# dy-tea/zpaq-v

Hardware: AMD Instinct MI355X
Metric: MB/s (comp+decomp) on level-2 64KiB blocks (higher is better)
Workload: dtype int32; 1 GPU; level 2 (ICM16+ISSE16+ISSE16), 8192 x 65536 B blocks per GPU (C5's per-GPU share of 65536 blocks over 8 GPUs), one segment per block, classes b mod 4 = zeros/uniform/markov-text/periodic (SURVEY 8(d) generator, block b of the global batch on rank b mod N); blocks_per_gpu=8192, block_bytes=65536, level=2, parallelism=block b -> gpu b mod 1, no collective

## Files before the change

### include/zpaq_hip.h

```cpp
#ifndef ZPAQ_HIP_H
#define ZPAQ_HIP_H

#include <stddef.h>
#include <stdint.h>

#ifdef __cplusplus
extern "C" {
#endif

#define ZPQ_OK 0
#define ZPQ_E_NODEVICE (-1)
#define ZPQ_E_ARG (-2)
#define ZPQ_E_HEADER (-3)
#define ZPQ_E_TOOBIG (-4)
#define ZPQ_E_MIX_M0 (-5)
#define ZPQ_E_NOMEM (-6)
#define ZPQ_E_OVERFLOW (-7)
#define ZPQ_E_VMSTEPS (-8)
#define ZPQ_E_INTERNAL (-9)
#define ZPQ_E_CLOSED (-10)

#define ZPQ_VM_STEP_CAP (1u << 20)

#define ZPQ_FLAG_PP 1u
// ... 12 lines not shown
int zpq_model_ncomp(const zpq_model *);
uint64_t zpq_model_state_bytes(const zpq_model *);
int zpq_model_has_fast_path(const zpq_model *);

typedef struct zpq_ctx zpq_ctx;
int zpq_ctx_create(int device, zpq_ctx **out);
void zpq_ctx_destroy(zpq_ctx *);
int zpq_ctx_sync(zpq_ctx *);
void *zpq_ctx_stream(zpq_ctx *);
int zpq_ctx_device(const zpq_ctx *);
int zpq_ctx_set_state_budget(zpq_ctx *, uint64_t bytes);
int zpq_ctx_set_max_block_bytes(zpq_ctx *, uint64_t bytes);
int zpq_ctx_last_slots(const zpq_ctx *);
unsigned zpq_ctx_last_host_transfer(const zpq_ctx *);
unsigned zpq_ctx_last_line_store(const zpq_ctx *);
int zpq_ctx_resident_capacity(zpq_ctx *, const zpq_model *, uint32_t flags);
float zpq_ctx_last_kernel_ms(const zpq_ctx *);
const char *zpq_ctx_last_kernel_name(const zpq_ctx *);

int zpq_encode_blocks(zpq_ctx *, const zpq_model *, int nblocks, const uint8_t *in,
                      const uint64_t *in_off, uint32_t flags, uint8_t *out,
                      const uint64_t *out_off, uint32_t *out_len, int32_t *status);
int zpq_decode_blocks(zpq_ctx *, const zpq_model *, int nblocks, const uint8_t *in,
                      const uint64_t *in_off, uint32_t flags, uint8_t *out,
                      const uint64_t *out_off, uint32_t *out_len, uint32_t *consumed,
                      uint32_t *final_code, uint32_t *first_byte, int32_t *status);

void *zpq_host_alloc(size_t bytes);
void zpq_host_free(void *);

// ... 76 lines not shown
```

### zpaq-v_amd/binding.py

```python
import atexit
import ctypes as C
import os
import weakref

import numpy as np

HERE = os.path.dirname(os.path.abspath(__file__))
FLAG_PP = 1
FLAG_GENERIC = 2
FLAG_LANES = 8
FLAG_VMPIPE = 16
SET_LANES = 1
SET_PIPE = 4
SET_WAVES = 16
SET_VMWAVES = 64
_LIB = None
_LIVE_CTX = weakref.WeakSet()
_LIVE_PINNED = weakref.WeakSet()
_FINALIZING = False


def _shutdown():
    global _FINALIZING
    for ctx in list(_LIVE_CTX):
# ... 42 lines not shown
    L.zpq_model_state_bytes.restype = u64
    L.zpq_model_has_fast_path.argtypes = [vp]
    L.zpq_ctx_create.argtypes = [i32, vp]
    L.zpq_ctx_destroy.argtypes = [vp]
    L.zpq_ctx_sync.argtypes = [vp]
    L.zpq_ctx_stream.argtypes = [vp]
    L.zpq_ctx_stream.restype = vp
    L.zpq_ctx_set_state_budget.argtypes = [vp, u64]
    L.zpq_ctx_set_max_block_bytes.argtypes = [vp, u64]
    L.zpq_ctx_last_slots.argtypes = [vp]
    L.zpq_ctx_last_host_transfer.argtypes = [vp]
    L.zpq_ctx_last_host_transfer.restype = C.c_uint
    L.zpq_ctx_last_line_store.argtypes = [vp]
    L.zpq_ctx_last_line_store.restype = C.c_uint
    L.zpq_ctx_resident_capacity.argtypes = [vp, vp, u32]
    L.zpq_ctx_last_kernel_ms.argtypes = [vp]
    L.zpq_ctx_last_kernel_ms.restype = C.c_float
    L.zpq_ctx_last_kernel_name.argtypes = [vp]
    L.zpq_ctx_last_kernel_name.restype = C.c_char_p
    enc = [vp, vp, i32, vp, vp, u32, vp, vp, vp, vp]
    dec = [vp, vp, i32, vp, vp, u32, vp, vp, vp, vp, vp, vp, vp]
    L.zpq_encode_blocks.argtypes = enc
    L.zpq_encode_blocks_dev.argtypes = enc
    L.zpq_decode_blocks.argtypes = dec
    L.zpq_decode_blocks_dev.argtypes = dec
    L.zpq_host_alloc.argtypes = [C.c_size_t]
    L.zpq_host_alloc.restype = vp
    L.zpq_host_free.argtypes = [vp]
    L.zpq_encode_blocks_multi.argtypes = [vp, i32, vp, i32, vp, vp, u32, vp, vp, vp, vp]
    L.zpq_decode_blocks_multi.argtypes = [vp, i32, vp, i32, vp, vp, u32, vp, vp, vp, vp, vp, vp, vp]
# ... 198 lines not shown
    def last_kernel_name(self):
        return lib().zpq_ctx_last_kernel_name(self.h).decode()

    @property
    def last_slots(self):
        return lib().zpq_ctx_last_slots(self.h)

    @property
    def last_host_transfer(self):
        return lib().zpq_ctx_last_host_transfer(self.h)

    @property
    def last_line_store(self):
        return lib().zpq_ctx_last_line_store(self.h)

    def resident_capacity(self, model, flags=FLAG_PP):
        n = lib().zpq_ctx_resident_capacity(self.h, model.h, flags)
        if n < 0:
            raise ZpqError(n, "zpq_ctx_resident_capacity")
        return n

    def blockset_capacity(self, model, max_member_bytes=0, lanes=False, pipe=False, waves=False, vmwaves=False):
        n = lib().zpq_blockset_capacity_ex(self.h, model.h, max_member_bytes, _set_flags(lanes, pipe, waves, vmwaves))
        if n < 0:
            raise ZpqError(n, "zpq_blockset_capacity")
        return n

    def encode_blocks(self, model, blocks, flags=FLAG_PP, cap=None):
        nb = len(blocks)
        in_off = _offsets([len(b) for b in blocks])
# ... 291 lines not shown
```

### zpaq-v_amd/csrc/zpq_api.hip

```cpp
#include <hip/hip_runtime.h>
#include <stdio.h>
#include <stdlib.h>
#include <string.h>
#include <time.h>

#include <algorithm>
#include <exception>
#include <map>
#include <mutex>
#include <thread>
#include <unordered_set>
#include <vector>

#include "../../include/zpaq_hip.h"
#include "zpq_common.h"
#include "zpq_host.h"

#define ZPQ_SET_ALL (ZPQ_SET_LANES | ZPQ_SET_PIPE | ZPQ_SET_WAVES | ZPQ_SET_VMWAVES)

#define HIPCK(x)                                                              \
    do {                                                                      \
        hipError_t e_ = (x);                                                  \
        if (e_ != hipSuccess) {                                               \
            fprintf(stderr, "[zpaq_hip] %s failed: %s (%s:%d)\n", #x, hipGetErrorString(e_), __FILE__, __LINE__); \
// ... 18 lines not shown
            (void)hipGetLastError();
            q = nullptr;
            if (p) { (void)hipFree(p); p = nullptr; cap = 0; }
            if (hipMalloc(&q, want) != hipSuccess) {
                (void)hipGetLastError();
                want = n + 4096;
                if (hipMalloc(&q, want) != hipSuccess) { (void)hipGetLastError(); return ZPQ_E_NOMEM; }
            }
        }
        if (p) (void)hipFree(p);
        p = q;
        cap = want;
        return ZPQ_OK;
    }
    void release() { if (p) (void)hipFree(p); p = nullptr; cap = 0; }
    DevBuf() = default;
    DevBuf(const DevBuf &) = delete;
    DevBuf &operator=(const DevBuf &) = delete;
    ~DevBuf() { release(); }
};

struct BlockArrays {
    int n = 0;
    const uint8_t *in = nullptr; const uint64_t *in_off = nullptr;
    uint32_t flags = 0;
    uint8_t *out = nullptr; const uint64_t *out_off = nullptr;
    uint32_t *out_len = nullptr, *consumed = nullptr, *final_code = nullptr, *first_byte = nullptr;
    int32_t *status = nullptr;
    BlockArrays window(int b0, int b1) const
    {
// ... 78 lines not shown
};

struct zpq_ctx {
    int device = 0;
    int cus = 256;
    hipStream_t stream = nullptr;
    hipEvent_t ev0 = nullptr, ev1 = nullptr;
    bool ev_valid = false;
    int16_t *d_squash = nullptr, *d_stretch = nullptr, *d_dt2k = nullptr;
    uint32_t *d_dt = nullptr, *d_stretch_c = nullptr;
    uint8_t *d_ns = nullptr;
    std::map<uint64_t, DevModel> models;
    uint32_t sparse_cap = 0;
    uint32_t sparse_pct = 112;
    DevBuf slots;
    uint64_t budget = 0;
    int last_slots = 0;
    unsigned last_host = 0;
    uint32_t last_sp = 0;
    const char *last_name = "";
    StageSet one, pipe[2];
    hipStream_t s_h2d = nullptr, s_d2h = nullptr;
    uint32_t *h_gate = nullptr;
    std::mutex mu;
    std::vector<zpq_block *> children;
    std::vector<zpq_blockset *> sets;
    uint64_t set_bytes = 0;
    uint64_t pool_budget() const { return budget > set_bytes ? budget - set_bytes : 0; }
};

// ... 35 lines not shown
    const zpq_model *model = nullptr;
    int nmembers = 0;
    bool chain = false;
    uint32_t flags = 0;
    uint32_t sp = 0;
    DModel layout;
    uint8_t *slots = nullptr;
    uint64_t bytes = 0;
    std::vector<int32_t> failed;
    std::vector<uint8_t> fresh;
    std::vector<uint8_t> open;
};

static int ctx_init(zpq_ctx *c, const zpq::Tables &T);
static int set_max_block_bytes(zpq_ctx *c, uint64_t bytes);
extern "C" int zpq_ctx_create(int device, zpq_ctx **out) try
{
    if (!out) return ZPQ_E_ARG;
    *out = nullptr;
    int ndev = 0;
    if (hipGetDeviceCount(&ndev) != hipSuccess || ndev <= 0) return ZPQ_E_NODEVICE;
    if (device < 0 || device >= ndev) return ZPQ_E_ARG;
    int tst = ZPQ_OK;
    const zpq::Tables &T = zpq::tables(&tst);
    if (tst != ZPQ_OK) return tst;
    HIPCK(hipSetDevice(device));
    zpq_ctx *c = new (std::nothrow) zpq_ctx();
    if (!c) return ZPQ_E_NOMEM;
    c->device = device;
    const int rc = ctx_init(c, T);
// ... 1 lines not shown
    if (rc != ZPQ_OK) { zpq_ctx_destroy(c); return rc; }
    *out = c;
    return ZPQ_OK;
} ZPQ_CATCH(return ZPQ_E_INTERNAL)

static int ctx_init(zpq_ctx *c, const zpq::Tables &T)
{
    const int device = c->device;
    hipDeviceProp_t prop;
    if (hipGetDeviceProperties(&prop, device) == hipSuccess) c->cus = prop.multiProcessorCount;
    HIPCK(hipStreamCreateWithFlags(&c->stream, hipStreamNonBlocking));
    HIPCK(hipEventCreate(&c->ev0));
    HIPCK(hipEventCreate(&c->ev1));
    HIPCK(hipStreamCreateWithFlags(&c->s_h2d, hipStreamNonBlocking));
    HIPCK(hipStreamCreateWithFlags(&c->s_d2h, hipStreamNonBlocking));
    HIPCK(hipHostMalloc((void **)&c->h_gate, 64, hipHostMallocPortable | hipHostMallocMapped));
    *c->h_gate = 1;
    for (auto &ps : c->pipe) if (int rc = ps.create_events()) return rc;
    std::vector<int16_t> sq(4096), st(32768), d2(256);
    for (int i = 0; i < 4096; i++) sq[i] = (int16_t)T.squash[i];
    for (int i = 0; i < 32768; i++) st[i] = (int16_t)T.stretch[i];
    for (int i = 0; i < 256; i++) d2[i] = (int16_t)T.dt2k[i];
    HIPCK(hipMalloc((void **)&c->d_squash, 4096 * 2));
    HIPCK(hipMalloc((void **)&c->d_stretch, 32768 * 2));
    HIPCK(hipMalloc((void **)&c->d_dt2k, 256 * 2));
    HIPCK(hipMalloc((void **)&c->d_dt, 1024 * 4));
    HIPCK(hipMalloc((void **)&c->d_ns, 1024));
    HIPCK(hipMalloc((void **)&c->d_stretch_c, sizeof T.stretch_c));
    HIPCK(hipMemcpy(c->d_squash, sq.data(), 4096 * 2, hipMemcpyHostToDevice));
    HIPCK(hipMemcpy(c->d_stretch, st.data(), 32768 * 2, hipMemcpyHostToDevice));
// ... 9 lines not shown
        const int pct = ev ? atoi(ev) : 0;
        if (pct >= 101 && pct <= 400) c->sparse_pct = (uint32_t)pct;
    }
    set_max_block_bytes(c, 65536);
    return ZPQ_OK;
}

extern "C" void zpq_ctx_destroy(zpq_ctx *c) try
{
    {
        std::lock_guard<std::mutex> lk(g_reg_mu);
        if (!c || !live_set().erase(c)) return;
    }
    (void)hipSetDevice(c->device);
    if (c->stream) (void)hipStreamSynchronize(c->stream);
    {
        std::lock_guard<std::mutex> lk(g_reg_mu);
        for (zpq_block *b : c->children) {
            if (b->slot) (void)hipFree(b->slot);
            b->slot = nullptr;
            b->ctx = nullptr;
        }
        c->children.clear();
        for (zpq_blockset *bs : c->sets) {
            if (bs->slots) (void)hipFree(bs->slots);
            bs->slots = nullptr;
            bs->ctx = nullptr;
        }
        c->sets.clear();
        c->set_bytes = 0;
    }
    for (auto &kv : c->models) { (void)hipFree(kv.second.d_model); (void)hipFree(kv.second.d_img); }
    if (c->h_gate) (void)hipHostFree(c->h_gate);
    if (c->s_h2d) { (void)hipStreamSynchronize(c->s_h2d); (void)hipStreamDestroy(c->s_h2d); }
    if (c->s_d2h) { (void)hipStreamSynchronize(c->s_d2h); (void)hipStreamDestroy(c->s_d2h); }
    (void)hipFree(c->d_squash); (void)hipFree(c->d_stretch); (void)hipFree(c->d_dt2k);
    (void)hipFree(c->d_dt); (void)hipFree(c->d_ns); (void)hipFree(c->d_stretch_c);
    if (c->ev0) (void)hipEventDestroy(c->ev0);
    if (c->ev1) (void)hipEventDestroy(c->ev1);
    if (c->stream) (void)hipStreamDestroy(c->stream);
    delete c;
} ZPQ_CATCH(return)

extern "C" int zpq_ctx_sync(zpq_ctx *c) try
{
    if (!ctx_live(c)) return ZPQ_E_ARG;
    HIPCK(hipStreamSynchronize(c->stream));
    return ZPQ_OK;
} ZPQ_CATCH(return ZPQ_E_INTERNAL)
extern "C" int zpq_ctx_device(const zpq_ctx *c) { return ctx_live(c) ? c->device : -1; }
extern "C" void *zpq_ctx_stream(zpq_ctx *c) { return ctx_live(c) ? (void *)c->stream : nullptr; }
extern "C" int zpq_ctx_set_state_budget(zpq_ctx *c, uint64_t bytes) try
{
    if (!ctx_live(c)) return ZPQ_E_ARG;
    c->budget = bytes;
    return ZPQ_OK;
} ZPQ_CATCH(return ZPQ_E_INTERNAL)
extern "C" int zpq_ctx_set_max_block_bytes(zpq_ctx *c, uint64_t bytes) try
{
    if (!ctx_live(c)) return ZPQ_E_ARG;
    return set_max_block_bytes(c, bytes);
} ZPQ_CATCH(return ZPQ_E_INTERNAL)
static uint32_t line_store_cap(const zpq_ctx *c, uint64_t bytes)
{
    const uint64_t probes = 2 * (bytes + 2);
    uint64_t cap = (probes * c->sparse_pct + 99) / 100 + 16;
    cap = (cap + 3) & ~3ull;
    if (cap > (1ull << 25)) cap = 1ull << 25;
    return (uint32_t)cap;
}
static int set_max_block_bytes(zpq_ctx *c, uint64_t bytes)
{
    c->sparse_cap = line_store_cap(c, bytes);
    return ZPQ_OK;
}
// ... 20 lines not shown
    HIPCK(hipMalloc((void **)&dm.d_img, m->img.size() * 4 + 4));
    HIPCK(hipMemcpy(dm.d_model, &layout, sizeof(DModel), hipMemcpyHostToDevice));
    HIPCK(hipMemcpy(dm.d_img, m->img.data(), m->img.size() * 4, hipMemcpyHostToDevice));
    c->models[key] = dm;
    *out = dm;
    return ZPQ_OK;
}

struct BatchArgs {
    BlockArrays io;
    BatchExtras x;
    const uint32_t *gate_flag = nullptr;
    uint32_t gate_pos = 0;
    uint32_t *prog_counter = nullptr;
    uint32_t prog_pos = 0;
};

static bool request(const char *var, uint32_t flags, uint32_t bit)
{
    const char *ev = getenv(var);
    const bool env = ev && (ev[0] == '0' || ev[0] == '1');
    return env ? ev[0] == '1' : (flags & bit) != 0;
}
struct SparseKnobs {
    uint32_t forced_cap = 0;
    bool never = false, always = false;
};
static SparseKnobs sparse_knobs()
{
    SparseKnobs k;
// ... 147 lines not shown
    if (rc != ZPQ_OK) return rc;
    c->last_name = name;
    HIPCK(hipGetLastError());
    HIPCK(hipEventRecord(c->ev1, s));
    c->ev_valid = true;
    return ZPQ_OK;
}
static int launch_family(zpq_ctx *c, const DBatch &B, const Plan &P, int decode, hipStream_t s)
{
    return timed_launch(c, s, [&](const char **name) {
        *name = FAMILY[P.fam].name[decode];
        return FAMILY[P.fam].launch(&B, P, decode, s, name);
    });
}

static int run_batch(zpq_ctx *c, const zpq_model *m, int decode, const BatchArgs &a)
{
    const BlockArrays &io = a.io;
    if (!ctx_live(c)) return c ? ZPQ_E_CLOSED : ZPQ_E_ARG;
    if (!m) return ZPQ_E_ARG;
    if (io.n < 0) return ZPQ_E_ARG;
    if (io.n == 0) return ZPQ_OK;
    if (!io.in_off || !io.out_off || !io.out_len || !io.status) return ZPQ_E_ARG;
    if (a.x.own_slot && io.n != 1) return ZPQ_E_ARG;
    HIPCK(hipSetDevice(c->device));
    Plan P;
    int rc = plan_batch(c, m, io.flags, io.n, a.x.trace != nullptr, a.x.own_slot != nullptr, &P, decode);
    if (rc != ZPQ_OK) return rc;
    DevModel dm;
    rc = get_dev_model(c, m, P.M, P.sp, &dm);
    if (rc != ZPQ_OK) return rc;

    DBatch B = batch_base(c, dm, io);
    B.trace = a.x.trace; B.ntrace = a.x.ntrace; B.ctx_out = a.x.ctx_out;
    B.gate_flag = (P.fam == F_CHAIN && !decode) ? a.gate_flag : nullptr;
    B.gate_pos = a.gate_pos;
    if (a.gate_flag && !B.gate_flag) return ZPQ_E_INTERNAL;
    B.prog_counter = (P.fam == F_CHAIN && decode) ? a.prog_counter : nullptr;
    B.prog_pos = a.prog_pos;

    if (a.x.own_slot) {
        B.slots = a.x.own_slot;
    } else {
        rc = c->slots.ensure((size_t)P.nslots * P.M.slot_bytes + 256);
        if (rc != ZPQ_OK) return rc;
        B.slots = (uint8_t *)c->slots.p;
    }
    B.nslots = P.nslots;
    c->last_slots = P.nslots;
    c->last_sp = P.sp;
    c->last_host = 0;
    return launch_family(c, B, P, decode, c->stream);
}

extern "C" int zpq_encode_blocks_dev(zpq_ctx *c, const zpq_model *m, int nblocks, const uint8_t *in,
                                     const uint64_t *in_off, uint32_t flags, uint8_t *out,
                                     const uint64_t *out_off, uint32_t *out_len, int32_t *status) try
{
    BatchArgs a;
    a.io = block_arrays(nblocks, in, in_off, flags & 0xffu, out, out_off, out_len, status);
    return run_batch(c, m, 0, a);
} ZPQ_CATCH(return ZPQ_E_INTERNAL)

extern "C" int zpq_decode_blocks_dev(zpq_ctx *c, const zpq_model *m, int nblocks, const uint8_t *in,
                                     const uint64_t *in_off, uint32_t flags, uint8_t *out,
                                     const uint64_t *out_off, uint32_t *out_len, uint32_t *consumed,
                                     uint32_t *final_code, uint32_t *first_byte, int32_t *status) try
{
    BatchArgs a;
    a.io = block_arrays(nblocks, in, in_off, flags & 0xffu, out, out_off, out_len, status, consumed, final_code, first_byte);
    return run_batch(c, m, 1, a);
} ZPQ_CATCH(return ZPQ_E_INTERNAL)

static int stage_room(StageSet &S, int nb, size_t in_bytes, size_t out_bytes, size_t misc_bytes)
{
    int rc;
    const size_t offb = (size_t)(nb + 1) * 8, u32b = (size_t)nb * 4;
    if ((rc = S.in.ensure(in_bytes + 16)) || (rc = S.out.ensure(out_bytes + 16)) || (rc = S.inoff.ensure(offb)) ||
        (rc = S.outoff.ensure(offb)) || (rc = S.dstoff.ensure(offb)) || (rc = S.meta.ensure(u32b * 4)) || (rc = S.status.ensure(u32b)) ||
        (rc = S.misc.ensure(misc_bytes)) || (rc = S.ensure_host((size_t)nb)))
        return rc;
    return ZPQ_OK;
}
static void stage_offsets(StageSet &S, const BlockArrays &h)
{
// ... 570 lines not shown
    if (!ctx_live(c)) return c ? ZPQ_E_CLOSED : ZPQ_E_ARG;
    if (!m || nmembers < 1) return ZPQ_E_ARG;
    HIPCK(hipSetDevice(c->device));
    std::lock_guard<std::mutex> lk(c->mu);
    zpq_blockset *s = new (std::nothrow) zpq_blockset();
    if (!s) return ZPQ_E_NOMEM;
    s->chain = set_layout(c, m, max_member_bytes, &s->layout, &s->sp);
    s->flags = (uint32_t)zpq_blockset_resolve_flags(m, flags);
    const bool lanes = (s->flags & ZPQ_SET_LANES) != 0;
    s->nmembers = nmembers;
    s->bytes = (uint64_t)nmembers * s->layout.slot_bytes + 256;
    if (nmembers > set_capacity(c, s->layout, s->chain, lanes) || s->bytes > c->pool_budget()) { delete s; return ZPQ_E_NOMEM; }
    if (hipMalloc((void **)&s->slots, s->bytes) != hipSuccess) {
        (void)hipGetLastError();
        (void)hipStreamSynchronize(c->stream);
        c->slots.release();
        if (hipMalloc((void **)&s->slots, s->bytes) != hipSuccess) { (void)hipGetLastError(); delete s; return ZPQ_E_NOMEM; }
    }
    int rc = ZPQ_OK;
    if (s->chain || lanes) {
        DevModel dm;
        rc = get_dev_model(c, m, s->layout, s->sp, &dm);
        if (rc == ZPQ_OK) rc = zpq_launch_lanes_set_init(dm.d_model, dm.d_img, s->slots, nmembers, c->stream);
        if (rc == ZPQ_OK && (hipGetLastError() != hipSuccess || hipStreamSynchronize(c->stream) != hipSuccess)) rc = ZPQ_E_NODEVICE;
    }
    if (rc != ZPQ_OK) { (void)hipGetLastError(); (void)hipFree(s->slots); delete s; return rc; }
    s->failed.assign((size_t)nmembers, ZPQ_OK);
    s->fresh.assign((size_t)nmembers, 1);
    s->open.assign((size_t)nmembers, 0);
    s->ctx = c; s->model = m;
// ... 251 lines not shown
```

### zpaq-v_amd/csrc/zpq_chain.hip

```cpp
#include <hip/hip_runtime.h>
#include <stdlib.h>
#include <string.h>

#include <type_traits>
#include <vector>

#include "../../include/zpaq_hip.h"
#include "zpq_common.h"
#include "zpq_vm.h"
#include "zpq_host.h"
#include "zpq_chain_cfg.h"
#include "zpq_dev.h"

constexpr int CHAIN_G_DEFAULT = 8;
constexpr bool CHAIN_SPEC_ENC = true, CHAIN_SPEC_DEC = false;

namespace zpqc {

using namespace zpqdev;
__device__ __forceinline__ i32 mul24x(i32 a, i32 b) { return __mul24(a, b); }

__device__ __forceinline__ i32 row_shr1(i32 self)
{
    return __builtin_amdgcn_update_dpp(self, self, 0x111 , 0xf, 0xf, false);
// ... 136 lines not shown
                        const u32 cmi = cmk[i] & 0x7FFFFFu;
                        const i32 sti = stretch_of(cmi);
                        d32[i] = cmi | (((u32)sti & 0x1FFu) << 23);
                        d8[i] = (u8)(sti >> 9);
                    } else {
                        const u32 a0 = cmk[2 * i], a1 = cmk[2 * i + 1];
                        d32[i] = (a0 & 0xFFFFFu) | (a1 << 20);
                        d8[i] = (u8)((i32)a1 >> 12);
                    }
                }
            }
        } else {
            uint4 *z4 = reinterpret_cast<uint4 *>(slot);
            const u64 n16 = M.zero_bytes / 16;
            const uint4 zero = make_uint4(0, 0, 0, 0);
            for (u64 i = li; i < n16; i += G) z4[i] = zero;
            for (int c = 0; c < n; c++) {
                const DComp &cc = M.comp[c];
                u32 *d32 = reinterpret_cast<u32 *>(my + cfg.lds_off32[c]);
                if (cc.type == ZT_ICM) {
                    u8 *d8 = my + cfg.lds_off8[c];
                    for (int i = li; i < 256; i += G) {
                        const u32 cmi = B.img[i];
                        const i32 sti = stretch_of(cmi);
                        d32[i] = cmi | (((u32)sti & 0x1FFu) << 23);
                        d8[i] = (u8)(sti >> 9);
                    }
                }
                else if (cc.type == ZT_ISSE) {
                    u8 *d8 = my + cfg.lds_off8[c];
                    for (int i = li; i < 256; i += G) {
// ... 1230 lines not shown
```

### zpaq-v_amd/csrc/zpq_common.h

```cpp
#pragma once
#include <stdint.h>

#define ZPQ_MAX_HDR 4096
#define ZPQ_MAX_COMP 255

enum { ZT_NONE = 0, ZT_CONST = 1, ZT_CM = 2, ZT_ICM = 3, ZT_MATCH = 4, ZT_AVG = 5,
       ZT_MIX2 = 6, ZT_MIX = 7, ZT_ISSE = 8, ZT_SSE = 9 };

enum { ZF_ZERO = 0, ZF_CONST = 1, ZF_PATTERN = 2 };

struct DComp {
    int32_t type;
    int32_t a, b, c, limit;
    int32_t j, k, rate, mask;
    uint32_t cm_len, ht_len, a16_len;
    uint32_t cm_fill, cm_fill_val, cm_pat_len;
    uint32_t a16_fill;
    uint32_t sp_cap;
    uint64_t cm_off, ht_off, a16_off;
    uint64_t sp_tag_off, sp_line_off;
};

struct DCompScal {
    int32_t a, b, c, limit;
// ... 15 lines not shown
    uint64_t regs_off, r_off, scal_off, h_off, m_off;
    uint64_t zero_bytes;
    uint64_t slot_bytes;
    uint32_t img_words;
    uint32_t pad_;
    uint8_t header[ZPQ_MAX_HDR];
    DComp comp[ZPQ_MAX_COMP];
};

struct DBatch {
    const DModel *model;
    const uint32_t *img;
    uint8_t *slots;
    int32_t nslots, nblocks;
    uint32_t flags;
    uint32_t ntrace;
    const uint8_t *in;
    const uint64_t *in_off;
    uint8_t *out;
    const uint64_t *out_off;
    uint32_t *out_len;
    uint32_t *consumed;
    uint32_t *final_code;
    uint32_t *first_byte;
    int32_t *status;
    union {
        int32_t *trace;
        const int32_t *slot_map;
    };
    uint32_t *ctx_out;
    const int16_t *squash;
// ... 23 lines not shown
```

### zpaq-v_amd/csrc/zpq_host.h

```cpp
#pragma once
#include <hip/hip_runtime.h>
#include <stdint.h>

#include <atomic>
#include <vector>

#include "zpq_common.h"

namespace zpq {

struct Tables {
    int32_t squash[4096];
    int32_t stretch[32768];
    int32_t dt[1024];
    int32_t dt2k[256];
    uint8_t ns[1024];
    uint32_t stretch_c[2048 + 128];
};
const Tables &tables(int *status);
uint64_t tables_fnv(int which);

}

bool zpq_sparse_layout(const DModel &dense, uint32_t cap, DModel *out);
// ... 32 lines not shown
int zpq_gdec_shape_applies(const DModel *M);
int zpq_gpipe_applies(const DModel *M);
int zpq_gpipe_blocks_per_cu(const DModel *M);
int zpq_launch_gpipe(const DBatch *B, const DModel *hostM, int nslots, hipStream_t stream);
int zpq_gdec_applies(const DModel *M);
int zpq_gdec_blocks_per_cu(const DModel *M);
int zpq_launch_gdec(const DBatch *B, const DModel *hostM, int nslots, hipStream_t stream);
int zpq_vpipe_applies(const DModel *M);
int zpq_vpipe_blocks_per_cu(const DModel *M);
int zpq_launch_vpipe(const DBatch *B, const DModel *hostM, int nslots, hipStream_t stream);
int zpq_vdec_applies(const DModel *M);
int zpq_vdec_blocks_per_cu(const DModel *M);
int zpq_launch_vdec(const DBatch *B, const DModel *hostM, int nslots, hipStream_t stream);
int zpq_launch_wset(const DBatch *B, const DModel *hostM, int decode, hipStream_t stream, const char **name);
int zpq_launch_vset(const DBatch *B, const DModel *hostM, int decode, hipStream_t stream, const char **name);
int zpq_launch_sha1(const uint8_t *in, const uint64_t *beg, const uint64_t *end, int n, uint8_t *out20, hipStream_t stream);
}

void zpq_note_exception(const char *where) noexcept;
#define ZPQ_CATCH(on_error) catch (...) { zpq_note_exception(__func__); on_error; }

template <class R, class F> static inline R zpq_guard(R on_error, const char *where, F &&f) noexcept
{
    try { return f(); } catch (...) { zpq_note_exception(where); return on_error; }
}
template <class F> static inline void zpq_guard_v(const char *where, F &&f) noexcept
{
    try { f(); } catch (...) { zpq_note_exception(where); }
}
```

### zpaq-v_amd/csrc/zpq_pipe.hip

```cpp
#include <hip/hip_runtime.h>
#include <stdlib.h>
#include <string.h>

#include <type_traits>

#include "../../include/zpaq_hip.h"
#include "zpq_common.h"
#include "zpq_chain_cfg.h"
#include "zpq_dev.h"
#include "zpq_host.h"

namespace zpqp {

using namespace zpqc;
using namespace zpqdev;

__device__ __forceinline__ bool gate_wait(const uint32_t *flag)
{
    u32 tries = 0;
    while (__hip_atomic_load(flag, __ATOMIC_ACQUIRE, __HIP_MEMORY_SCOPE_SYSTEM) == 0u) {
        __builtin_amdgcn_s_sleep(64);
        if (++tries > (1u << 22)) return false;
    }
    return true;
// ... 867 lines not shown
                    reinterpret_cast<u32 *>(blk_lds + cfg.lds_off32[0])[i] = cmi | (((u32)sti & 0x1FFu) << 23);
                    (blk_lds + cfg.lds_off8[0])[i] = (u8)(sti >> 9);
                }
#pragma unroll 1
                for (int c = 1; c < NCH; c++) {
                    const u32 *cmk = reinterpret_cast<const u32 *>(bslot + M.comp[c].cm_off);
                    const u32 a0 = cmk[2 * i], a1 = cmk[2 * i + 1];
                    reinterpret_cast<u32 *>(blk_lds + cfg.lds_off32[c])[i] = (a0 & 0xFFFFFu) | (a1 << 20);
                    (blk_lds + cfg.lds_off8[c])[i] = (u8)((i32)a1 >> 12);
                }
            }
            if (tid == 0) *misc = 0u;
        } else {
            const u64 n16 = M.zero_bytes / 16;
            const uint4 zero = make_uint4(0, 0, 0, 0);
            for (int b = 0; b < nact; b++) {
                uint4 *z4 = reinterpret_cast<uint4 *>(B.slots + (u64)(wg_slot0 + b) * M.slot_bytes);
                for (u64 i = tid; i < n16; i += nthr) z4[i] = zero;
            }
            for (int idx = tid; idx < nact * 256; idx += nthr) {
                const int b = idx >> 8, i = idx & 255;
                u8 *blk_lds = lds + LDS_STATE + b * cfg.lds_per_block;
                {
                    const u32 cmi = B.img[i];
                    u32 q = cmi >> 8;
                    q = min(max(q, 1u), 32767u);
                    const u32 wv = s_stretch[q >> 4];
                    const u32 ei = q < 64u ? q : (q - 32704u + 64u);
                    const i32 endv = (i32)(int16_t)s_stretch[2048 + (ei & 127u)];
                    const i32 midv = (i32)(int16_t)(wv >> 16) + __popc(wv & ((2u << (q & 15u)) - 1u) & 0xFFFEu);
                    const i32 sti = (q < 64u || q >= 32704u) ? endv : midv;
// ... 108 lines not shown
        int o = -1;
        for (int c = 0; c < NCH; c++) {
            if ((split_mask >> c) & 1) { dP[c] = o + 1 < 1 ? 1 : o + 1; dH[c] = dP[c] - 1; o = dP[c]; }
            else { dP[c] = o + 1; dH[c] = dP[c]; o = dP[c]; }
        }
        dC = o + 1;
    }

    for (int base = wg_slot0; base < B.nblocks; base += nslots) {
        const int blk = base + lane;
        const bool active = lane_on && blk < B.nblocks;
        const int nact = min(wg_slots, B.nblocks - base);
        {
            const u64 n16 = M.zero_bytes / 16;
            const uint4 zero = make_uint4(0, 0, 0, 0);
            for (int b = 0; b < nact; b++) {
                uint4 *z4 = reinterpret_cast<uint4 *>(B.slots + (u64)(wg_slot0 + b) * M.slot_bytes);
                for (u64 i = tid; i < n16; i += nthr) z4[i] = zero;
            }
            for (int idx = tid; idx < nact * 256; idx += nthr) {
                const int b = idx >> 8, i = idx & 255;
                u8 *blk_lds = lds + LDS_STATE + b * cfg.lds_per_block;
                {
                    const u32 cmi = B.img[i];
                    u32 q = cmi >> 8;
                    q = min(max(q, 1u), 32767u);
                    const u32 wv = s_stretch[q >> 4];
                    const u32 ei = q < 64u ? q : (q - 32704u + 64u);
                    const i32 endv = (i32)(int16_t)s_stretch[2048 + (ei & 127u)];
                    const i32 midv = (i32)(int16_t)(wv >> 16) + __popc(wv & ((2u << (q & 15u)) - 1u) & 0xFFFEu);
                    const i32 sti = (q < 64u || q >= 32704u) ? endv : midv;
// ... 215 lines not shown
```

Baseline: 1525 MB/s.

## Zero encode slots with a low-priority janitor during decode via a spare pool

Decode batches now run in a separately allocated spare slot buffer. A low-priority stream meanwhile runs a throttled janitor kernel that re-zeroes the encode slot buffer left dirty by the previous encode. A small policy state machine records that the slots are clean for the same model layout, so the next encode kernel skips per-slot zeroing for the first nclean slots. The intent is to move the model-state zeroing off the critical path of encode. The cost is an extra device allocation sized to the slot pool, cross-stream event dependencies, and contention from the janitor stealing bandwidth from decode.

```diff
diff --git a/include/zpaq_hip.h b/include/zpaq_hip.h
--- a/include/zpaq_hip.h
+++ b/include/zpaq_hip.h
@@ -50,6 +50,7 @@
 int zpq_ctx_last_slots(const zpq_ctx *);
 unsigned zpq_ctx_last_host_transfer(const zpq_ctx *);
 unsigned zpq_ctx_last_line_store(const zpq_ctx *);
+int zpq_ctx_spare_stats(zpq_ctx *, uint64_t out[4]);
 int zpq_ctx_resident_capacity(zpq_ctx *, const zpq_model *, uint32_t flags);
 float zpq_ctx_last_kernel_ms(const zpq_ctx *);
 const char *zpq_ctx_last_kernel_name(const zpq_ctx *);
diff --git a/zpaq-v_amd/binding.py b/zpaq-v_amd/binding.py
--- a/zpaq-v_amd/binding.py
+++ b/zpaq-v_amd/binding.py
@@ -80,6 +80,8 @@
     L.zpq_ctx_last_line_store.argtypes = [vp]
     L.zpq_ctx_last_line_store.restype = C.c_uint
     L.zpq_ctx_resident_capacity.argtypes = [vp, vp, u32]
+    if hasattr(L, "zpq_ctx_spare_stats"):
+        L.zpq_ctx_spare_stats.argtypes = [vp, vp]
     L.zpq_ctx_last_kernel_ms.argtypes = [vp]
     L.zpq_ctx_last_kernel_ms.restype = C.c_float
     L.zpq_ctx_last_kernel_name.argtypes = [vp]
@@ -308,6 +310,12 @@
     def last_line_store(self):
         return lib().zpq_ctx_last_line_store(self.h)
 
+    @property
+    def spare_stats(self):
+        out = (C.c_uint64 * 4)()
+        _ck(lib().zpq_ctx_spare_stats(self.h, out), "zpq_ctx_spare_stats")
+        return dict(zip(("janitor_launches", "slots_cleaned", "slots_skipped", "spare_bytes"), (int(v) for v in out)))
+
     def resident_capacity(self, model, flags=FLAG_PP):
         n = lib().zpq_ctx_resident_capacity(self.h, model.h, flags)
         if n < 0:
diff --git a/zpaq-v_amd/csrc/zpq_api.hip b/zpaq-v_amd/csrc/zpq_api.hip
--- a/zpaq-v_amd/csrc/zpq_api.hip
+++ b/zpaq-v_amd/csrc/zpq_api.hip
@@ -56,6 +56,13 @@
         return ZPQ_OK;
     }
     void release() { if (p) (void)hipFree(p); p = nullptr; cap = 0; }
+    int exact(size_t n)
+    {
+        release();
+        if (hipMalloc(&p, n) != hipSuccess) { (void)hipGetLastError(); p = nullptr; return ZPQ_E_NOMEM; }
+        cap = n;
+        return ZPQ_OK;
+    }
     DevBuf() = default;
     DevBuf(const DevBuf &) = delete;
     DevBuf &operator=(const DevBuf &) = delete;
@@ -164,6 +171,13 @@
     uint32_t sparse_cap = 0;
     uint32_t sparse_pct = 112;
     DevBuf slots;
+    DevBuf spare;
+    zpq_spare_state sp = {};
+    hipStream_t s_jan = nullptr;
+    hipEvent_t ev_enc = nullptr, ev_jan = nullptr;
+    bool jan_pending = false;
+    uint64_t jan_slot_bytes = 0, jan_zero_bytes = 0;
+    uint64_t sp_stats[4] = {0, 0, 0, 0};
     uint64_t budget = 0;
     int last_slots = 0;
     unsigned last_host = 0;
@@ -229,6 +243,7 @@
 
 static int ctx_init(zpq_ctx *c, const zpq::Tables &T);
 static int set_max_block_bytes(zpq_ctx *c, uint64_t bytes);
+static void spare_reset(zpq_ctx *c);
 extern "C" int zpq_ctx_create(int device, zpq_ctx **out) try
 {
     if (!out) return ZPQ_E_ARG;
@@ -260,6 +275,13 @@
     HIPCK(hipEventCreate(&c->ev1));
     HIPCK(hipStreamCreateWithFlags(&c->s_h2d, hipStreamNonBlocking));
     HIPCK(hipStreamCreateWithFlags(&c->s_d2h, hipStreamNonBlocking));
+    {
+        int lo = 0, hi = 0;
+        if (hipDeviceGetStreamPriorityRange(&lo, &hi) != hipSuccess) { (void)hipGetLastError(); lo = 0; }
+        HIPCK(hipStreamCreateWithPriority(&c->s_jan, hipStreamNonBlocking, lo));
+    }
+    HIPCK(hipEventCreateWithFlags(&c->ev_enc, hipEventDisableTiming));
+    HIPCK(hipEventCreateWithFlags(&c->ev_jan, hipEventDisableTiming));
     HIPCK(hipHostMalloc((void **)&c->h_gate, 64, hipHostMallocPortable | hipHostMallocMapped));
     *c->h_gate = 1;
     for (auto &ps : c->pipe) if (int rc = ps.create_events()) return rc;
@@ -299,6 +321,7 @@
     }
     (void)hipSetDevice(c->device);
     if (c->stream) (void)hipStreamSynchronize(c->stream);
+    if (c->s_jan) (void)hipStreamSynchronize(c->s_jan);
     {
         std::lock_guard<std::mutex> lk(g_reg_mu);
         for (zpq_block *b : c->children) {
@@ -323,6 +346,9 @@
     (void)hipFree(c->d_dt); (void)hipFree(c->d_ns); (void)hipFree(c->d_stretch_c);
     if (c->ev0) (void)hipEventDestroy(c->ev0);
     if (c->ev1) (void)hipEventDestroy(c->ev1);
+    if (c->ev_enc) (void)hipEventDestroy(c->ev_enc);
+    if (c->ev_jan) (void)hipEventDestroy(c->ev_jan);
+    if (c->s_jan) (void)hipStreamDestroy(c->s_jan);
     if (c->stream) (void)hipStreamDestroy(c->stream);
     delete c;
 } ZPQ_CATCH(return)
@@ -331,6 +357,7 @@
 {
     if (!ctx_live(c)) return ZPQ_E_ARG;
     HIPCK(hipStreamSynchronize(c->stream));
+    HIPCK(hipStreamSynchronize(c->s_jan));
     return ZPQ_OK;
 } ZPQ_CATCH(return ZPQ_E_INTERNAL)
 extern "C" int zpq_ctx_device(const zpq_ctx *c) { return ctx_live(c) ? c->device : -1; }
@@ -339,11 +366,13 @@
 {
     if (!ctx_live(c)) return ZPQ_E_ARG;
     c->budget = bytes;
+    spare_reset(c);
     return ZPQ_OK;
 } ZPQ_CATCH(return ZPQ_E_INTERNAL)
 extern "C" int zpq_ctx_set_max_block_bytes(zpq_ctx *c, uint64_t bytes) try
 {
     if (!ctx_live(c)) return ZPQ_E_ARG;
+    spare_reset(c);
     return set_max_block_bytes(c, bytes);
 } ZPQ_CATCH(return ZPQ_E_INTERNAL)
 static uint32_t line_store_cap(const zpq_ctx *c, uint64_t bytes)
@@ -394,6 +423,7 @@
     uint32_t gate_pos = 0;
     uint32_t *prog_counter = nullptr;
     uint32_t prog_pos = 0;
+    bool spare_ok = false;
 };
 
 static bool request(const char *var, uint32_t flags, uint32_t bit)
@@ -571,6 +601,129 @@
     });
 }
 
+#define SPARE_POOL_DEFAULT 1
+struct JanitorKnobs { bool enabled; unsigned burst, nap; int waves; };
+static JanitorKnobs janitor_knobs()
+{
+    JanitorKnobs k = {SPARE_POOL_DEFAULT != 0, 8u, 16u, -1};
+    const char *ev = getenv("ZPQ_SPARE_POOL");
+    if (ev && (ev[0] == '0' || ev[0] == '1')) k.enabled = ev[0] == '1';
+    if ((ev = getenv("ZPQ_JANITOR_BURST")) && atoi(ev) >= 1 && atoi(ev) <= 4096) k.burst = (unsigned)atoi(ev);
+    if ((ev = getenv("ZPQ_JANITOR_NAP")) && atoi(ev) >= 0 && atoi(ev) <= 65536) k.nap = (unsigned)atoi(ev);
+    if ((ev = getenv("ZPQ_JANITOR_WAVES")) && atoi(ev) >= 0 && atoi(ev) <= 4096) k.waves = atoi(ev);
+    return k;
+}
+static bool spare_layout_ok(const Plan &P, uint32_t flags)
+{
+    if (P.fam != F_CHAIN || P.sp != 0 || (flags & (ZB_KEEP_STATE | ZB_CHUNK))) return false;
+    for (int i = 0; i < P.M.n; i++) if (P.M.comp[i].type == ZT_MIX2 || P.M.comp[i].sp_cap) return false;
+    return P.M.zero_bytes != 0 && (P.M.zero_bytes & 15) == 0 && P.M.zero_bytes <= P.M.slot_bytes;
+}
+static void spare_signature(const DModel &M, uint64_t sig[ZPQ_SPARE_SIG])
+{
+    uint64_t h = 0xcbf29ce484222325ull;
+    auto mix = [&](uint64_t v) { for (int i = 0; i < 8; i++) { h ^= (v >> (8 * i)) & 255u; h *= 0x100000001b3ull; } };
+    mix(M.regs_off); mix(M.r_off); mix(M.scal_off); mix(M.h_off); mix(M.m_off); mix(M.mlen); mix(M.hlen);
+    for (int i = 0; i < M.n; i++) {
+        const DComp &C = M.comp[i];
+        mix((uint64_t)C.type); mix(C.cm_off); mix(C.ht_off); mix(C.a16_off); mix(C.cm_len); mix(C.ht_len); mix(C.a16_len);
+    }
+    sig[0] = M.slot_bytes; sig[1] = M.zero_bytes; sig[2] = (uint64_t)M.n; sig[3] = h;
+}
+static void spare_drop(zpq_ctx *c)
+{
+    if (c->s_jan) (void)hipStreamSynchronize(c->s_jan);
+    c->jan_pending = false;
+    if (c->spare.p) { if (c->stream) (void)hipStreamSynchronize(c->stream); c->spare.release(); }
+}
+static void spare_reset(zpq_ctx *c)
+{
+    (void)hipSetDevice(c->device);
+    (void)zpq_spare_policy(&c->sp, ZPQ_SPARE_EV_RESET, nullptr, 0, 0, 0, 0, 1);
+    spare_drop(c);
+}
+static int spare_before_launch(zpq_ctx *c, const Plan &P, int decode, bool eligible, size_t need, DBatch *B, bool *janitor)
+{
+    const JanitorKnobs K = janitor_knobs();
+    uint64_t sig[ZPQ_SPARE_SIG];
+    spare_signature(P.M, sig);
+    *janitor = false;
+    bool in_spare = false;
+    if (eligible && decode) {
+        size_t fr = 0, tot = 0;
+        const bool may_alloc = K.enabled && !c->sp.have_spare && c->sp.e_state == ZPQ_SPARE_E_USED;
+        if (may_alloc && hipMemGetInfo(&fr, &tot) != hipSuccess) { (void)hipGetLastError(); fr = 0; }
+        const size_t margin = 256u << 20;
+        int v = zpq_spare_policy(&c->sp, ZPQ_SPARE_EV_DECODE, sig, P.nslots, need, c->pool_budget(), fr > margin ? fr - margin : 0, K.enabled);
+        if (v & ZPQ_SPARE_DO_DROP) spare_drop(c);
+        if ((v & ZPQ_SPARE_DO_ALLOC) && c->spare.exact(need) != ZPQ_OK) {
+            (void)zpq_spare_policy(&c->sp, ZPQ_SPARE_EV_RESET, nullptr, 0, 0, 0, 0, 1);
+            v = 0;
+        }
+        in_spare = (v & ZPQ_SPARE_DO_DECODE_IN_D) != 0;
+        *janitor = (v & ZPQ_SPARE_DO_JANITOR) != 0;
+    }
+    if (in_spare) {
+        if (need > c->spare.cap) return ZPQ_E_INTERNAL;
+        B->slots = (uint8_t *)c->spare.p;
+        return ZPQ_OK;
+    }
+    if (need > c->slots.cap && (c->sp.have_spare || c->jan_pending)) spare_reset(c);
+    if (!(eligible && !decode)) (void)zpq_spare_policy(&c->sp, ZPQ_SPARE_EV_OTHER, nullptr, 0, 0, 0, 0, K.enabled);
+    if (c->jan_pending) {
+        HIPCK(hipStreamWaitEvent(c->stream, c->ev_jan, 0));
+        c->jan_pending = false;
+    }
+    if (eligible && !decode) {
+        const int v = zpq_spare_policy(&c->sp, ZPQ_SPARE_EV_ENCODE, sig, P.nslots, need, 0, 0, K.enabled);
+        if (v & ZPQ_SPARE_DO_DROP) spare_drop(c);
+        if (v & ZPQ_SPARE_DO_SKIP) {
+            B->nclean = (uint32_t)c->sp.skip_slots;
+            c->sp_stats[2] += (uint64_t)c->sp.skip_slots;
+        }
+        c->jan_slot_bytes = P.M.slot_bytes; c->jan_zero_bytes = P.M.zero_bytes;
+    } else if (!K.enabled && c->spare.p) spare_drop(c);
+    const int rc = c->slots.ensure(need);
+    if (rc != ZPQ_OK) return rc;
+    B->slots = (uint8_t *)c->slots.p;
+    return ZPQ_OK;
+}
+static void spare_after_launch(zpq_ctx *c, int decode, bool in_pool, bool janitor)
+{
+    if (!decode && in_pool && c->sp.e_state == ZPQ_SPARE_E_USED) {
+        if (hipEventRecord(c->ev_enc, c->stream) != hipSuccess) {
+            (void)hipGetLastError();
+            (void)zpq_spare_policy(&c->sp, ZPQ_SPARE_EV_OTHER, nullptr, 0, 0, 0, 0, 1);
+        }
+        return;
+    }
+    if (!janitor) return;
+    const JanitorKnobs K = janitor_knobs();
+    const int ns = c->sp.e_slots;
+    const int waves = K.waves < 0 ? c->cus : K.waves;
+    bool ok = waves > 0 && ns > 0 && c->jan_slot_bytes && (uint64_t)ns * c->jan_slot_bytes <= c->slots.cap;
+    ok = ok && hipStreamWaitEvent(c->s_jan, c->ev_enc, 0) == hipSuccess;
+    ok = ok && zpq_launch_janitor((uint8_t *)c->slots.p, c->jan_slot_bytes, c->jan_zero_bytes, ns, waves, K.burst, K.nap, c->s_jan) == ZPQ_OK;
+    if (ok) c->jan_pending = true;
+    ok = ok && hipEventRecord(c->ev_jan, c->s_jan) == hipSuccess;
+    if (!ok) {
+        (void)hipGetLastError();
+        if (c->jan_pending) { (void)hipStreamSynchronize(c->s_jan); c->jan_pending = false; }
+        (void)zpq_spare_policy(&c->sp, ZPQ_SPARE_EV_OTHER, nullptr, 0, 0, 0, 0, 1);
+        return;
+    }
+    c->sp_stats[0] += 1;
+    c->sp_stats[1] += (uint64_t)ns;
+}
+
+extern "C" int zpq_ctx_spare_stats(zpq_ctx *c, uint64_t out[4]) try
+{
+    if (!ctx_live(c) || !out) return ZPQ_E_ARG;
+    for (int i = 0; i < 3; i++) out[i] = c->sp_stats[i];
+    out[3] = c->spare.p ? (uint64_t)c->spare.cap : 0;
+    return ZPQ_OK;
+} ZPQ_CATCH(return ZPQ_E_INTERNAL)
+
 static int run_batch(zpq_ctx *c, const zpq_model *m, int decode, const BatchArgs &a)
 {
     const BlockArrays &io = a.io;
@@ -582,6 +735,7 @@
     if (a.x.own_slot && io.n != 1) return ZPQ_E_ARG;
     HIPCK(hipSetDevice(c->device));
     Plan P;
+    bool janitor = false;
     int rc = plan_batch(c, m, io.flags, io.n, a.x.trace != nullptr, a.x.own_slot != nullptr, &P, decode);
     if (rc != ZPQ_OK) return rc;
     DevModel dm;
@@ -599,15 +753,19 @@
     if (a.x.own_slot) {
         B.slots = a.x.own_slot;
     } else {
-        rc = c->slots.ensure((size_t)P.nslots * P.M.slot_bytes + 256);
+        const size_t need = (size_t)P.nslots * P.M.slot_bytes + 256;
+        const bool eligible = a.spare_ok && !a.gate_flag && !a.prog_counter && spare_layout_ok(P, io.flags);
+        rc = spare_before_launch(c, P, decode, eligible, need, &B, &janitor);
         if (rc != ZPQ_OK) return rc;
-        B.slots = (uint8_t *)c->slots.p;
     }
     B.nslots = P.nslots;
     c->last_slots = P.nslots;
     c->last_sp = P.sp;
     c->last_host = 0;
-    return launch_family(c, B, P, decode, c->stream);
+    rc = launch_family(c, B, P, decode, c->stream);
+    if (rc != ZPQ_OK) return rc;
+    if (!a.x.own_slot) spare_after_launch(c, decode, B.slots == (uint8_t *)c->slots.p, janitor);
+    return ZPQ_OK;
 }
 
 extern "C" int zpq_encode_blocks_dev(zpq_ctx *c, const zpq_model *m, int nblocks, const uint8_t *in,
@@ -616,6 +774,7 @@
 {
     BatchArgs a;
     a.io = block_arrays(nblocks, in, in_off, flags & 0xffu, out, out_off, out_len, status);
+    a.spare_ok = true;
     return run_batch(c, m, 0, a);
 } ZPQ_CATCH(return ZPQ_E_INTERNAL)
 
@@ -626,6 +785,7 @@
 {
     BatchArgs a;
     a.io = block_arrays(nblocks, in, in_off, flags & 0xffu, out, out_off, out_len, status, consumed, final_code, first_byte);
+    a.spare_ok = true;
     return run_batch(c, m, 1, a);
 } ZPQ_CATCH(return ZPQ_E_INTERNAL)
 
@@ -1226,6 +1386,7 @@
     if (hipMalloc((void **)&s->slots, s->bytes) != hipSuccess) {
         (void)hipGetLastError();
         (void)hipStreamSynchronize(c->stream);
+        spare_reset(c);
         c->slots.release();
         if (hipMalloc((void **)&s->slots, s->bytes) != hipSuccess) { (void)hipGetLastError(); delete s; return ZPQ_E_NOMEM; }
     }
diff --git a/zpaq-v_amd/csrc/zpq_chain.hip b/zpaq-v_amd/csrc/zpq_chain.hip
--- a/zpaq-v_amd/csrc/zpq_chain.hip
+++ b/zpaq-v_amd/csrc/zpq_chain.hip
@@ -174,7 +174,12 @@
             uint4 *z4 = reinterpret_cast<uint4 *>(slot);
             const u64 n16 = M.zero_bytes / 16;
             const uint4 zero = make_uint4(0, 0, 0, 0);
-            for (u64 i = li; i < n16; i += G) z4[i] = zero;
+            if constexpr (DEC || SP || MIXT) {
+                for (u64 i = li; i < n16; i += G) z4[i] = zero;
+            } else {
+                if (blk != slot_id || (u32)slot_id >= B.nclean)
+                    for (u64 i = li; i < n16; i += G) z4[i] = zero;
+            }
             for (int c = 0; c < n; c++) {
                 const DComp &cc = M.comp[c];
                 u32 *d32 = reinterpret_cast<u32 *>(my + cfg.lds_off32[c]);
diff --git a/zpaq-v_amd/csrc/zpq_common.h b/zpaq-v_amd/csrc/zpq_common.h
--- a/zpaq-v_amd/csrc/zpq_common.h
+++ b/zpaq-v_amd/csrc/zpq_common.h
@@ -53,7 +53,10 @@
     uint8_t *slots;
     int32_t nslots, nblocks;
     uint32_t flags;
-    uint32_t ntrace;
+    union {
+        uint32_t ntrace;
+        uint32_t nclean;
+    };
     const uint8_t *in;
     const uint64_t *in_off;
     uint8_t *out;
diff --git a/zpaq-v_amd/csrc/zpq_host.h b/zpaq-v_amd/csrc/zpq_host.h
--- a/zpaq-v_amd/csrc/zpq_host.h
+++ b/zpaq-v_amd/csrc/zpq_host.h
@@ -70,6 +70,22 @@
 int zpq_launch_vdec(const DBatch *B, const DModel *hostM, int nslots, hipStream_t stream);
 int zpq_launch_wset(const DBatch *B, const DModel *hostM, int decode, hipStream_t stream, const char **name);
 int zpq_launch_vset(const DBatch *B, const DModel *hostM, int decode, hipStream_t stream, const char **name);
+int zpq_launch_janitor(uint8_t *slots, uint64_t slot_bytes, uint64_t zero_bytes, int nslots, int waves, unsigned burst, unsigned nap,
+                       hipStream_t stream);
+#define ZPQ_SPARE_SIG 4
+enum { ZPQ_SPARE_E_UNKNOWN = 0, ZPQ_SPARE_E_USED = 1, ZPQ_SPARE_E_CLEAN = 2 };
+enum { ZPQ_SPARE_EV_ENCODE = 0, ZPQ_SPARE_EV_DECODE = 1, ZPQ_SPARE_EV_OTHER = 2, ZPQ_SPARE_EV_RESET = 3 };
+enum { ZPQ_SPARE_DO_SKIP = 1, ZPQ_SPARE_DO_ALLOC = 2, ZPQ_SPARE_DO_DECODE_IN_D = 4, ZPQ_SPARE_DO_JANITOR = 8, ZPQ_SPARE_DO_DROP = 16 };
+struct zpq_spare_state {
+    uint64_t layout[ZPQ_SPARE_SIG];
+    uint64_t spare_bytes;
+    int32_t have_spare;
+    int32_t e_state;
+    int32_t e_slots;
+    int32_t skip_slots;
+};
+int zpq_spare_policy(zpq_spare_state *S, int event, const uint64_t layout[ZPQ_SPARE_SIG], int nslots, uint64_t need_bytes,
+                     uint64_t budget_bytes, uint64_t free_bytes, int enabled);
 int zpq_launch_sha1(const uint8_t *in, const uint64_t *beg, const uint64_t *end, int n, uint8_t *out20, hipStream_t stream);
 }
 
diff --git a/zpaq-v_amd/csrc/zpq_janitor.hip b/zpaq-v_amd/csrc/zpq_janitor.hip
--- /dev/null
+++ b/zpaq-v_amd/csrc/zpq_janitor.hip
@@ -0,0 +1,96 @@
+#include <hip/hip_runtime.h>
+#include <stdint.h>
+#include <string.h>
+
+#include "../../include/zpaq_hip.h"
+#include "zpq_host.h"
+
+namespace zpqj {
+
+typedef uint64_t u64;
+typedef uint32_t u32;
+
+__global__ void __launch_bounds__(64) k_janitor(uint8_t *slots, u64 slot_bytes, u64 n16, u32 nslot, u32 burst, u32 nap)
+{
+    const u64 rows_per_slot = (n16 + 63) / 64;
+    const u64 total = rows_per_slot * nslot;
+    const u64 nburst = (total + burst - 1) / burst;
+    typedef u32 v4u __attribute__((ext_vector_type(4)));
+    const v4u zero = {0u, 0u, 0u, 0u};
+    for (u64 q = blockIdx.x; q < nburst; q += gridDim.x) {
+        const u64 r0 = q * burst;
+        u64 s = r0 / rows_per_slot, row = r0 - s * rows_per_slot;
+        const u32 nrow = (u32)(total - r0 < burst ? total - r0 : burst);
+        for (u32 k = 0; k < nrow; k++) {
+            const u64 i = row * 64 + threadIdx.x;
+            v4u *const p = reinterpret_cast<v4u *>(slots + s * slot_bytes) + i;
+            if (i < n16) *p = zero;
+            if (++row == rows_per_slot) { row = 0; s++; }
+        }
+        for (u32 k = 0; k < nap; k++) __builtin_amdgcn_s_sleep(4);
+    }
+}
+
+}
+
+extern "C" int zpq_launch_janitor(uint8_t *slots, uint64_t slot_bytes, uint64_t zero_bytes, int nslots, int waves,
+                                  unsigned burst, unsigned nap, hipStream_t stream)
+{
+    if (!slots || nslots <= 0 || waves <= 0 || zero_bytes > slot_bytes || (zero_bytes & 15) || (slot_bytes & 15)) return ZPQ_E_INTERNAL;
+    if (burst < 1) burst = 1;
+    if (burst > 4096) burst = 4096;
+    if (nap > 65536) nap = 65536;
+    hipLaunchKernelGGL(zpqj::k_janitor, dim3(waves), dim3(64), 0, stream, slots, slot_bytes, zero_bytes / 16, (uint32_t)nslots, burst, nap);
+    return hipGetLastError() == hipSuccess ? ZPQ_OK : ZPQ_E_NODEVICE;
+}
+
+extern "C" int zpq_spare_policy(zpq_spare_state *S, int event, const uint64_t layout[ZPQ_SPARE_SIG], int nslots,
+                                uint64_t need_bytes, uint64_t budget_bytes, uint64_t free_bytes, int enabled)
+{
+    if (!S) return 0;
+    int verdict = 0;
+    auto same = [&](void) { return layout && memcmp(S->layout, layout, sizeof S->layout) == 0; };
+    auto drop = [&](void) { S->have_spare = 0; S->spare_bytes = 0; };
+    if (!enabled && event != ZPQ_SPARE_EV_RESET) {
+        if (S->have_spare) verdict |= ZPQ_SPARE_DO_DROP;
+        drop();
+        S->e_state = ZPQ_SPARE_E_UNKNOWN; S->e_slots = 0;
+        return verdict;
+    }
+    switch (event) {
+    case ZPQ_SPARE_EV_ENCODE:
+        if (S->e_state == ZPQ_SPARE_E_CLEAN && same() && nslots > 0) {
+            verdict |= ZPQ_SPARE_DO_SKIP;
+            S->skip_slots = S->e_slots < nslots ? S->e_slots : nslots;
+        } else S->skip_slots = 0;
+        if (layout) memcpy(S->layout, layout, sizeof S->layout);
+        S->e_state = ZPQ_SPARE_E_USED; S->e_slots = nslots;
+        break;
+    case ZPQ_SPARE_EV_DECODE:
+        if (!S->have_spare && S->e_state == ZPQ_SPARE_E_USED) {
+            const bool fits = need_bytes && need_bytes <= budget_bytes / 2 && need_bytes <= free_bytes;
+            if (fits) { verdict |= ZPQ_SPARE_DO_ALLOC; S->have_spare = 1; S->spare_bytes = need_bytes; }
+        } else if (S->have_spare && need_bytes > S->spare_bytes) {
+            verdict |= ZPQ_SPARE_DO_DROP;
+            drop();
+        }
+        if (S->have_spare) {
+            verdict |= ZPQ_SPARE_DO_DECODE_IN_D;
+            if (S->e_state == ZPQ_SPARE_E_USED && S->e_slots > 0) {
+                verdict |= ZPQ_SPARE_DO_JANITOR;
+                S->e_state = ZPQ_SPARE_E_CLEAN;
+            }
+        } else { S->e_state = ZPQ_SPARE_E_UNKNOWN; S->e_slots = 0; }
+        break;
+    case ZPQ_SPARE_EV_OTHER:
+        S->e_state = ZPQ_SPARE_E_UNKNOWN; S->e_slots = 0;
+        break;
+    case ZPQ_SPARE_EV_RESET:
+    default:
+        if (S->have_spare) verdict |= ZPQ_SPARE_DO_DROP;
+        drop();
+        S->e_state = ZPQ_SPARE_E_UNKNOWN; S->e_slots = 0;
+        break;
+    }
+    return verdict;
+}
diff --git a/zpaq-v_amd/csrc/zpq_pipe.hip b/zpaq-v_amd/csrc/zpq_pipe.hip
--- a/zpaq-v_amd/csrc/zpq_pipe.hip
+++ b/zpaq-v_amd/csrc/zpq_pipe.hip
@@ -905,7 +905,8 @@
         } else {
             const u64 n16 = M.zero_bytes / 16;
             const uint4 zero = make_uint4(0, 0, 0, 0);
-            for (int b = 0; b < nact; b++) {
+            const int nskip = (MIXT || SP) ? 0 : (base == wg_slot0 ? min(max((int)B.nclean - wg_slot0, 0), nact) : 0);
+            for (int b = nskip; b < nact; b++) {
                 uint4 *z4 = reinterpret_cast<uint4 *>(B.slots + (u64)(wg_slot0 + b) * M.slot_bytes);
                 for (u64 i = tid; i < n16; i += nthr) z4[i] = zero;
             }
@@ -1044,7 +1045,8 @@
         {
             const u64 n16 = M.zero_bytes / 16;
             const uint4 zero = make_uint4(0, 0, 0, 0);
-            for (int b = 0; b < nact; b++) {
+            const int nskip = base == wg_slot0 ? min(max((int)B.nclean - wg_slot0, 0), nact) : 0;
+            for (int b = nskip; b < nact; b++) {
                 uint4 *z4 = reinterpret_cast<uint4 *>(B.slots + (u64)(wg_slot0 + b) * M.slot_bytes);
                 for (u64 i = tid; i < n16; i += nthr) z4[i] = zero;
             }
```

Measured after the change: 1544 MB/s (median of 6 runs). +1.2%, better.
